# mfinzi/depth-estimation

Hardware: AMD Instinct MI355X
Metric: Mpixel-labels/s per CRF mean-field iter (splat+blur+slice) (higher is better)
Workload: dtype f32; 1 GPU; c3: synthetic 2048x1536x256 cost volume, d=5 bilateral features (BASELINE configs[2]); H=1536, W=2048, L=256, d=5, features=synthetic smooth colours sigma_xy=8.0 sigma_c=0.1, n=3145728, M=296893, parallelism=single GPU, launch=eager, arithmetic=default (fp32-rounding-equivalent, ~1e-7 rel), table=reference

## Files before the change

### depth-estimation_amd/csrc/phl_api.hip

```cpp
#include <math.h>
#include <stdarg.h>
#include <stdio.h>
#include <string.h>

#include <map>
#include <chrono>
#include <mutex>
#include <utility>
#include <vector>

#include "phl_internal.h"

namespace {
thread_local char g_err[512] = "";

struct device_guard {
    int prev = -1;
    bool ok = false;
    explicit device_guard(int dev)
    {
        if (hipGetDevice(&prev) != hipSuccess) prev = -1;
        ok = (prev == dev) || (hipSetDevice(dev) == hipSuccess);
    }
    ~device_guard()
// ... 757 lines not shown
int phl_splat_part_pack(phl_lattice *lat, const float *src, int vd, int64_t src_rs, float *vert, float *partial_dev,
                        const int32_t *chunks_dev, int64_t nchunks_sel, const int32_t *rows_dev, int64_t nrows,
                        const int32_t *pack_pos_dev, float *pack_dev, int64_t pack_rs, phl_stream st)
{
    if (!lat || vd < 0 || nchunks_sel < 0 || nrows < 0 || !vert || (nchunks_sel > 0 && (!chunks_dev || !src)) || (nrows > 0 && !rows_dev) ||
        (lat->S_multi > 0 && !partial_dev) || (pack_pos_dev && (!pack_dev || pack_rs < vd || pack_rs % 4 || !phl_al16(pack_dev)))) {
        phl_set_error("phl_splat_part_pack: bad arguments");
        return PHL_ERR_INVALID;
    }
    return splat_subset("phl_splat_part_pack", lat, src, vd, src_rs, vert, partial_dev, chunks_dev, nchunks_sel, rows_dev, nrows,
                        pack_pos_dev, pack_dev, pack_rs, st);
}

int phl_blur_axis(phl_lattice *lat, int axis, const float *vin, float *vout, int vd, phl_stream st)
{
    if (!lat || axis < 0 || axis > lat->d || vd < 0 || vin == vout) { phl_set_error("phl_blur_axis: bad arguments"); return PHL_ERR_INVALID; }
    device_guard g(lat->device);
    return phl_launch_blur(lat, axis, vin, vout, vd, (hipStream_t)st);
}

static int blur_all(const phl_lattice *lat, float *const buf[2], int vd, hipStream_t st, int *cur_out)
{
    static const bool pairs = !(getenv("PHL_BLUR_PAIRS") && atoi(getenv("PHL_BLUR_PAIRS")) == 0);
    int cur = 0;
    for (int axis = 0; axis <= lat->d;) {
        int rc;
        if (pairs && axis + 1 <= lat->d && lat->nbr2) {
            rc = phl_launch_blur2(lat, axis / 2, buf[cur], buf[cur ^ 1], vd, st, true);
            axis += 2;
        } else {
            rc = phl_launch_blur(lat, axis, buf[cur], buf[cur ^ 1], vd, st, true);
            axis += 1;
        }
        if (rc) return rc;
        cur ^= 1;
    }
    *cur_out = cur;
    return PHL_OK;
}

int phl_blur(phl_lattice *lat, float *vert_a, float *vert_b, int vd, int *result_in_b, phl_stream st)
{
    if (!lat || vd < 0 || !result_in_b || vert_a == vert_b || (lat->M > 0 && vd > 0 && (!vert_a || !vert_b))) {
        phl_set_error("phl_blur: bad arguments");
        return PHL_ERR_INVALID;
    }
    device_guard g(lat->device);
// ... 229 lines not shown
    if (lat->M == 0) return PHL_OK;
    device_guard g(lat->device);
    PHL_HIP(hipDeviceSynchronize());
    std::vector<int32_t> f, r;
    int rc = fetch_maps(lat, f, r);
    if (rc) return rc;
    const size_t M = (size_t)lat->M;
    const int axes = lat->d + 1;
    if (r.empty()) {
        PHL_HIP(hipMemcpy(nbr, lat->nbr, sizeof(int32_t) * M * axes * 2, hipMemcpyDeviceToHost));
        return PHL_OK;
    }
    std::vector<int32_t> h(M * axes * 2);
    PHL_HIP(hipMemcpy(h.data(), lat->nbr, sizeof(int32_t) * h.size(), hipMemcpyDeviceToHost));
    for (int a = 0; a < axes; a++)
        for (size_t v = 0; v < M; v++)
            for (int s2 = 0; s2 < 2; s2++) {
                const int32_t x = h[((size_t)a * M + r[v]) * 2 + s2];
                nbr[((size_t)a * M + v) * 2 + s2] = x < 0 ? x : f[x];
            }
    return PHL_OK;
}

int phl_get_splat_lists(phl_lattice *lat, int32_t *ptr, int32_t *pixel, float *w)
{
    if (!lat || !ptr || !pixel || !w) { phl_set_error("phl_get_splat_lists: bad arguments"); return PHL_ERR_INVALID; }
    if (lat->N == 0) { ptr[0] = 0; return PHL_OK; }
    device_guard g(lat->device);
    const int rc0 = phl_ensure_csr(lat, nullptr);
    if (rc0) return rc0;
    std::vector<phl_contrib_t> h((size_t)lat->N);
    std::vector<int32_t> p((size_t)lat->M + 1);
    PHL_HIP(hipDeviceSynchronize());
    PHL_HIP(hipMemcpy(p.data(), lat->csr_ptr, sizeof(int32_t) * p.size(), hipMemcpyDeviceToHost));
    PHL_HIP(hipMemcpy(h.data(), lat->csr, sizeof(phl_contrib_t) * h.size(), hipMemcpyDeviceToHost));
    std::vector<int32_t> f, r;
    int rc = fetch_maps(lat, f, r);
    if (rc) return rc;
    int64_t o = 0;
    for (int64_t v = 0; v < lat->M; v++) {
        const int64_t row = r.empty() ? v : r[v];
        ptr[v] = (int32_t)o;
        for (int32_t e = p[row]; e < p[row + 1]; e++, o++) { pixel[o] = h[e].pixel; w[o] = h[e].w; }
    }
    ptr[lat->M] = (int32_t)o;
    return PHL_OK;
// ... 4 lines not shown
```

### depth-estimation_amd/csrc/phl_build.hip

```cpp
#include <cstring>
#include <mutex>

#include "phl_device_utils.h"

namespace {

struct sf_t {
    float v[PHL_MAX_D];
};

template <int D>
struct pix_rec {
    static constexpr int GW = (D + 1) / 2;
    static constexpr int W = GW + (D + 5) / 6;
    static __device__ __forceinline__ void load(const uint32_t *__restrict__ p, uint32_t (&w)[W])
    {
        if constexpr (W == 4) {
            const uint4 v = *reinterpret_cast<const uint4 *>(p);
            w[0] = v.x; w[1] = v.y; w[2] = v.z; w[3] = v.w;
        } else if constexpr (W == 2) {
            const uint2 v = *reinterpret_cast<const uint2 *>(p);
            w[0] = v.x; w[1] = v.y;
        } else {
#pragma unroll
// ... 392 lines not shown
        for (int side = 0; side < 2; side++) t[side] = open[side] ? table[h[side]] : PHL_EMPTY;
        uint32_t other[2][K::KW];
#pragma unroll
        for (int side = 0; side < 2; side++) {
            if (t[side] == PHL_EMPTY) { open[side] = false; continue; }
            K::load(vkp + (int64_t)(-(t[side] + 1)) * K::PW, other[side]);
        }
#pragma unroll
        for (int side = 0; side < 2; side++) {
            if (!open[side]) continue;
            bool same = true;
#pragma unroll
            for (int j = 0; j < K::KW; j++) same &= (other[side][j] == want[side][j]);
            if (same) { res[side] = -(t[side] + 1); open[side] = false; }
            else h[side] = (h[side] + 1) & mask;
        }
    }
    nbr[idx * 2 + 0] = res[0];
    nbr[idx * 2 + 1] = res[1];
}

template <int D>
int launch_neighbors(const int16_t *vkeys, int M, const int *table, uint32_t mask, int *nbr, phl_dev_block<uint32_t> &scratch,
                     hipStream_t st)
{
    using K = packed_key<D>;
    PHL_TRY(scratch.alloc((size_t)M * K::PW + 4));
    uint32_t *const vkp = scratch.get();
    hipLaunchKernelGGL(k_pack_keys<D>, dim3((M + 255) / 256), dim3(256), 0, st, vkeys, M, vkp);
    const int64_t tot = (int64_t)M * (D + 1);
    hipLaunchKernelGGL(k_neighbors<D>, dim3((unsigned)((tot + 255) / 256)), dim3(256), 0, st, vkp, M, table, mask, nbr);
    PHL_HIP(hipGetLastError());
    return PHL_OK;
}

__global__ __launch_bounds__(256) void k_compose_pairs(const int2 *__restrict__ nbr, int M, int npairs, int4 *__restrict__ nbr2)
{
    const int64_t idx = (int64_t)blockIdx.x * blockDim.x + threadIdx.x;
    if (idx >= (int64_t)M * npairs) return;
    const int p = (int)(idx / M);
    const int v = (int)(idx - (int64_t)p * M);
    const int2 *na = nbr + (int64_t)(2 * p) * M;
    const int2 nb = nbr[(int64_t)(2 * p + 1) * M + v];
    const int2 none = make_int2(-1, -1);
    const int2 am = nb.x >= 0 ? na[nb.x] : none;
    const int2 a0 = na[v];
    const int2 ap = nb.y >= 0 ? na[nb.y] : none;
    nbr2[idx * 2 + 0] = make_int4(am.x, nb.x, am.y, a0.x);
    nbr2[idx * 2 + 1] = make_int4(a0.y, ap.x, nb.y, ap.y);
}

struct hidden_t {
    int n;
    int32_t id[PHL_MAX_HIDDEN];
};

__global__ __launch_bounds__(256) void k_table_insert(const int16_t *__restrict__ vkeys, int d, int M, int *table,
                                                      uint32_t mask, hidden_t hidden, const int *__restrict__ int_of_ft)
{
    const int v = blockIdx.x * blockDim.x + threadIdx.x;
    if (v >= M) return;
    for (int i = 0; i < hidden.n; i++)
        if ((int_of_ft ? int_of_ft[hidden.id[i]] : hidden.id[i]) == v) return;
    const int16_t *key = vkeys + (int64_t)v * d;
    uint32_t h = mix_begin();
    for (int i = 0; i < d; i++) h = mix_step(h, key[i]);
    h = mix_end(h) & mask;
    while (atomicCAS(&table[h], PHL_EMPTY, -(v + 1)) != PHL_EMPTY) h = (h + 1) & mask;
}

__global__ __launch_bounds__(256) void k_table_lookup(const int16_t *__restrict__ qkeys, int d, int K,
                                                      const int16_t *__restrict__ vkeys, const int *__restrict__ table,
// ... 115 lines not shown

#define PHL_FOR_D(X)                                                                                                     \
    X(1) X(2) X(3) X(4) X(5) X(6) X(7) X(8) X(9) X(10) X(11) X(12) X(13) X(14) X(15) X(16)

__global__ __launch_bounds__(256) void k_iota_from(int *p, int n, int first)
{
    const int i = blockIdx.x * blockDim.x + threadIdx.x;
    if (i < n) p[i] = first + i;
}

__global__ void k_override_nbr00(int *nbr, const int *__restrict__ int_of_ft, int value)
{
    const int row = int_of_ft ? int_of_ft[0] : 0;
    nbr[(int64_t)row * 2] = (value >= 0 && int_of_ft) ? int_of_ft[value] : value;
}

}

int phl_rebuild_table_and_neighbors(phl_lattice *lat, hipStream_t st, phl_dev_block<uint32_t> &scratch)
{
    const int d = lat->d;
    const int M = (int)lat->M;
    PHL_HIP(phl_lat_free(lat->nbr2));
    uint64_t cap = 1024;
    while (cap < (uint64_t)M * 2) cap <<= 1;
    lat->table_mask = (uint32_t)(cap - 1);
    PHL_HIP(phl_lat_alloc(lat->table, cap));
    PHL_HIP(phl_lat_alloc(lat->nbr, (size_t)M * (d + 1) * 2));
    hipLaunchKernelGGL(k_fill_i32, dim3(1024), dim3(256), 0, st, lat->table, (int64_t)cap, PHL_EMPTY);
    if (M > 0) {
        hidden_t hidden;
        hidden.n = lat->n_hidden;
        for (int i = 0; i < lat->n_hidden; i++) hidden.id[i] = lat->hidden[i];
        hipLaunchKernelGGL(k_table_insert, dim3((M + 255) / 256), dim3(256), 0, st, lat->vkeys, d, M, lat->table,
                           lat->table_mask, hidden, lat->int_of_ft);
        int rcn = PHL_OK;
        switch (d) {
#define PHL_CASE(D) case D: rcn = launch_neighbors<D>(lat->vkeys, M, lat->table, lat->table_mask, lat->nbr, scratch, st); break;
            PHL_FOR_D(PHL_CASE)
#undef PHL_CASE
        }
        if (rcn) return rcn;
        if (lat->nbr00_override != -2)
            hipLaunchKernelGGL(k_override_nbr00, dim3(1), dim3(1), 0, st, lat->nbr, lat->int_of_ft, lat->nbr00_override);
        const int npairs = (d + 1) / 2;
        PHL_HIP(phl_lat_alloc(lat->nbr2, (size_t)M * npairs * 8));
        const int64_t totp = (int64_t)M * npairs;
        hipLaunchKernelGGL(k_compose_pairs, dim3((unsigned)((totp + 255) / 256)), dim3(256), 0, st,
                           reinterpret_cast<const int2 *>(lat->nbr), M, npairs, reinterpret_cast<int4 *>(lat->nbr2));
    }
    PHL_HIP(hipGetLastError());
    return PHL_OK;
}

int phl_write_final_vids(phl_lattice *lat, hipStream_t st)
{
    if (!lat->bt_slot_of || !lat->bt_table) { phl_set_error("phl_write_final_vids: no build tables"); return PHL_ERR_INVALID; }
    const int N = (int)lat->N;
    if (N > 0) {
        hipLaunchKernelGGL(k_final_vid, dim3((unsigned)(((int64_t)N + 256 * FV_PER - 1) / (256 * FV_PER))), dim3(256), 0, st, lat->bt_table, lat->bt_slot_of, N,
                           lat->bt_remap, lat->bt_dup_ptr, lat->bt_seg_e, lat->bt_seg_id, lat->int_of_ft, lat->replay);
        PHL_HIP(hipGetLastError());
    }
    return PHL_OK;
}

namespace {
struct side_t {
    int dev = -1;
    hipStream_t s = nullptr;
    hipEvent_t fork = nullptr, join = nullptr;
};
// ... 306 lines not shown
```

### depth-estimation_amd/csrc/phl_filter.hip

```cpp
#include <stdlib.h>

#include <type_traits>

#include "phl_internal.h"

namespace {

template <int VEC> struct vec_of;
template <> struct vec_of<1> { using type = float; };
template <> struct vec_of<4> { using type = float4; };

template <int VEC> __device__ __forceinline__ typename vec_of<VEC>::type vzero();
template <> __device__ __forceinline__ float vzero<1>() { return 0.f; }
template <> __device__ __forceinline__ float4 vzero<4>() { return make_float4(0.f, 0.f, 0.f, 0.f); }

__device__ __forceinline__ float vload(const float *p, float) { return *p; }
__device__ __forceinline__ float4 vload(const float *p, float4) { return *reinterpret_cast<const float4 *>(p); }
__device__ __forceinline__ void vstore(float *p, float v) { *p = v; }
__device__ __forceinline__ void vstore(float *p, float4 v) { *reinterpret_cast<float4 *>(p) = v; }

__device__ __forceinline__ float mac(float acc, float w, float q) { return acc + w * q; }
__device__ __forceinline__ float4 mac(float4 acc, float w, float4 q)
{
    return make_float4(acc.x + w * q.x, acc.y + w * q.y, acc.z + w * q.z, acc.w + w * q.w);
// ... 171 lines not shown
            s[u] = vload(vin + vc * vd + c, V());
#pragma unroll
            for (int k = 0; k < 8; k++) {
                if constexpr (LPR == 64) {
                    const int idk = __builtin_amdgcn_readfirstlane(id[u][k]);
                    x[u][k] = vzero<VEC>();
                    if (idk >= 0) x[u][k] = vload(vin + (int64_t)idk * vd + c, V());
                } else {
                    x[u][k] = vzero<VEC>();
                    if (__ballot(id[u][k] >= 0) != 0ull)
                        x[u][k] = vload(vin + (id[u][k] >= 0 ? (int64_t)id[u][k] : vc) * vd + c, V());
                }
            }
        }
#pragma unroll
        for (int u = 0; u < U; u++) {
#pragma unroll
            for (int k = 0; k < 8; k++)
                if (id[u][k] < 0) x[u][k] = vzero<VEC>();
            const V tm = id[u][1] >= 0 ? blur3(x[u][0], x[u][1], x[u][2]) : vzero<VEC>();
            const V t0 = blur3(x[u][3], s[u], x[u][4]);
            const V tp = id[u][6] >= 0 ? blur3(x[u][5], x[u][6], x[u][7]) : vzero<VEC>();
            if (v[u] < M) vstore(vout + v[u] * vd + c, blur3(tm, t0, tp));
        }
    }
}

template <int VEC, int LPR, bool EXACT>
__global__ __launch_bounds__(256) void k_slice(const float *__restrict__ vert, int vd,
                                               const phl_replay_t *__restrict__ replay, int dp1, int64_t n,
                                               float *__restrict__ out, int64_t out_rs,
                                               const float *__restrict__ sub_src, int64_t sub_rs, float cdiv,
                                               float rcdiv)
{
    using V = typename vec_of<VEC>::type;
    constexpr int G = 64 / LPR;
    const int lane = threadIdx.x & 63;
    const int sub = lane / LPR;
    const int l = lane % LPR;
    const int64_t stride = (int64_t)waves_in_grid() * G;
    for (int64_t p0 = (int64_t)wave_in_grid() * G; p0 < n; p0 += stride) {
        const int64_t p = p0 + sub;
        if (p >= n) continue;
        const phl_replay_t *rp = replay + p * dp1;
        for (int c = l * VEC; c < vd; c += LPR * VEC) {
            V acc = vzero<VEC>();
// ... 185 lines not shown
    });
    PHL_HIP(hipGetLastError());
    return PHL_OK;
}

int phl_launch_rows(bool scatter, float *vert, int vd, const int64_t *idx, int64_t k, float *buf, int64_t buf_rs, hipStream_t st)
{
    if (k == 0 || vd == 0) return PHL_OK;
    if (vd % 4 || buf_rs % 4 || !phl_al16(vert) || !phl_al16(buf)) {
        phl_set_error("row gather/scatter: needs vd %% 4 == 0 and 16-byte aligned rows");
        return PHL_ERR_UNSUPPORTED;
    }
    const int lpr = pick_lpr(vd, 4);
    const unsigned grid = (unsigned)((k + (64 / lpr) * 4 - 1) / ((64 / lpr) * 4));
    dispatch_int<PHL_LPRS>(lpr, [&](auto L) {
        constexpr int LPR = decltype(L)::value;
        if (scatter) k_scatter_add_rows<LPR><<<dim3(grid), dim3(256), 0, st>>>(vert, vd, idx, k, buf, buf_rs);
        else k_gather_rows<LPR><<<dim3(grid), dim3(256), 0, st>>>(vert, vd, idx, k, buf, buf_rs);
    });
    PHL_HIP(hipGetLastError());
    return PHL_OK;
}

int phl_launch_blur2(const phl_lattice *lat, int pair, const float *vin, float *vout, int vd, hipStream_t st, bool restricted)
{
    const int M = (int)lat->M;
    if (M == 0 || vd == 0) return PHL_OK;
    const blur_rows_t rr = rows_of(lat, 2 * pair + 1, restricted);
    if (rr.total == 0) return PHL_OK;
    const int4 *nb2 = reinterpret_cast<const int4 *>(lat->nbr2) + (int64_t)pair * M * 2;
    const bool v4 = (vd % 4 == 0) && phl_al16(vin) && phl_al16(vout);
    constexpr int U2 = 1;
    const row_launch rl = launch_rows(rr.total, vd, v4, U2);
    dispatch_int<PHL_LPRS>(rl.lpr, [&](auto L) {
        constexpr int LPR = decltype(L)::value;
        if (v4) k_blur2<4, LPR, U2><<<dim3(rl.grid), dim3(256), 0, st>>>(vin, vout, nb2, M, vd, rl.xcd_chunk, rr);
        else k_blur2<1, LPR, U2><<<dim3(rl.grid), dim3(256), 0, st>>>(vin, vout, nb2, M, vd, rl.xcd_chunk, rr);
    });
    PHL_HIP(hipGetLastError());
    return PHL_OK;
}

int phl_launch_slice(const phl_lattice *lat, const float *vert, int vd, float *out, int64_t out_rs, const float *sub,
                     int64_t sub_rs, unsigned flags, hipStream_t st)
{
    const int64_t n = lat->n;
    if (n == 0 || vd == 0) return PHL_OK;
    const int dp1 = lat->d + 1;
    const float cdiv = 1 + powf(2, -lat->d);
    const float rcdiv = 1.0f / cdiv;
    const bool v4 = (vd % 4 == 0) && (out_rs % 4 == 0) && phl_al16(vert) && phl_al16(out) &&
                    (!sub || ((sub_rs % 4 == 0) && phl_al16(sub)));
    const int lpr = pick_lpr(vd, v4 ? 4 : 1);
// ... 48 lines not shown
```

### depth-estimation_amd/csrc/phl_internal.h

```cpp
#pragma once
#include <hip/hip_runtime.h>
#include <stdint.h>
#include <stdlib.h>

#include "phl.h"

#include <type_traits>
#include <utility>
#include <vector>

#define PHL_WAVE 64
#define PHL_MAX_HIDDEN 64
#define PHL_EMPTY 0x7FFFFFFF

void phl_set_error(const char *fmt, ...);
int phl_hip_fail(hipError_t e, const char *what, const char *file, int line);
#define PHL_HIP(call)                                                              \
    do {                                                                           \
        hipError_t e__ = (call);                                                   \
        if (e__ != hipSuccess) return phl_hip_fail(e__, #call, __FILE__, __LINE__); \
    } while (0)
#define PHL_TRY(call) \
    do { const int rc__ = (call); if (rc__ != PHL_OK) return rc__; } while (0)

struct phl_replay_t {
    int32_t vid;
    float w;
};
struct phl_contrib_t {
    int32_t pixel;
    float w;
};

struct phl_lattice {
    int device;
    int d;
    int64_t n;
    int64_t M;
    int64_t N;

    int16_t *vkeys;
    phl_replay_t *replay;
    int32_t *csr_ptr;
    phl_contrib_t *csr;
    int32_t *nbr;
    int32_t *nbr2;
    int *table;
    uint32_t table_mask;
    int64_t M_local;
    int32_t *vfirst;
    int64_t vfirst_valid_for_M;
    int32_t *bt_slot_of, *bt_table;
    int32_t *bt_remap, *bt_dup_ptr, *bt_seg_e, *bt_seg_id;
    int32_t *bt_cell;
    int grid_nca, grid_ncb;
    int32_t *ft_of_int;
    int32_t *int_of_ft;

    int P;
    int nchunks;
    int nv_max;
    int64_t S;
    int64_t S_multi;
    int32_t *pix_order;
    int32_t *chunk_vptr;
    int32_t *slot_vert;
    int32_t *slot_pidx;
    int2 *seg_rng;
    phl_contrib_t *seg;
// ... 21 lines not shown
    int32_t nbr00_override;
};

hipError_t phl_dev_malloc(void **p, size_t bytes);
hipError_t phl_dev_free(void *p);

template <typename T>
inline hipError_t phl_lat_free(T *&member) { return phl_dev_free(std::exchange(member, nullptr)); }
template <typename T>
inline hipError_t phl_lat_alloc(T *&member, size_t count)
{
    hipError_t e = phl_lat_free(member);
    void *p = nullptr;
    if (e == hipSuccess) e = phl_dev_malloc(&p, sizeof(T) * (count ? count : (size_t)1));
    if (e == hipSuccess) member = (T *)p;
    return e;
}

template <typename... T>
inline void phl_lat_free_all(T *&...member) { ((void)phl_lat_free(member), ...); }
inline void phl_lat_free_persistent(phl_lattice *lat)
{
    phl_lat_free_all(lat->vkeys, lat->replay, lat->csr_ptr, lat->csr, lat->nbr, lat->nbr2, lat->table, lat->ft_of_int, lat->int_of_ft,
                     lat->vfirst);
}
inline void phl_tiles_free(phl_lattice *lat)
{
    phl_lat_free_all(lat->pix_order, lat->chunk_vptr, lat->slot_vert, lat->slot_pidx, lat->seg_rng, lat->seg, lat->lidx, lat->vs_ptr,
                     lat->vs, lat->vorder, lat->chunk_by_nv, lat->vlong);
    free(lat->nv_cum);
    lat->nv_cum = nullptr;
    lat->n_long = lat->S = lat->S_multi = 0;
    lat->nchunks = lat->nv_max = 0;
}
inline void phl_release_build_tables(phl_lattice *lat)
{
    phl_lat_free_all(lat->bt_slot_of, lat->bt_table, lat->bt_remap, lat->bt_dup_ptr, lat->bt_cell);
    lat->bt_seg_e = lat->bt_seg_id = nullptr;
}

struct phl_reftable_query {
    virtual int vid_at(int64_t candidate) = 0;
    virtual int64_t next_occurrence(int clean_vid, int64_t after) = 0;
    virtual void probe_paths_submit(int64_t n_clean, const std::vector<int32_t> &extra_clean,
                                    const std::vector<int32_t> &stale_clean, uint64_t cap,
                                    const std::vector<int32_t> &check) = 0;
    virtual int probe_paths_all_ok() = 0;
// ... 192 lines not shown
struct phl_splat_opts {
    bool subset = false;
    const int *chunk_list = nullptr;
    int nlist = 0;
    const int *vlist = nullptr;
    int64_t nvl = 0;
    const phl_splat_wide *wide = nullptr;
    const int *pack_pos = nullptr;
    float *pack = nullptr;
    int64_t pack_rs = 0;
};
int phl_launch_splat_tiled(phl_lattice *lat, const float *src, int64_t src_rs, int vd, float *vert, float *partial,
                           hipStream_t st, const phl_splat_opts &o = {});
int phl_launch_slice_grad(const phl_lattice *lat, const float *vertw, int L, const float *y, int64_t y_rs, const float *ref,
                          int64_t ref_rs, int64_t ref_cs, float *grad_ref, int k0, int ncols, int accumulate, float *wx_out,
                          int64_t wx_rs, hipStream_t st);
int phl_tiles_chunks_touching(phl_lattice *lat, const int64_t *rows_dev, int64_t k, int32_t *mask_host, hipStream_t st);
int phl_launch_slice_tiled(const phl_lattice *lat, const float *vert, int vd, float *out, int64_t out_rs, const float *sub,
                           int64_t sub_rs, unsigned flags, hipStream_t st);

int phl_launch_splat(phl_lattice *lat, const float *src, int64_t src_rs, int vd, float *vert, hipStream_t st);
int phl_launch_blur(const phl_lattice *lat, int axis, const float *vin, float *vout, int vd, hipStream_t st, bool restricted = false);
int phl_launch_blur2(const phl_lattice *lat, int pair, const float *vin, float *vout, int vd, hipStream_t st, bool restricted = false);
int phl_launch_rows(bool scatter, float *vert, int vd, const int64_t *idx, int64_t k, float *buf, int64_t buf_rs, hipStream_t st);
int phl_launch_slice(const phl_lattice *lat, const float *vert, int vd, float *out, int64_t out_rs,
                     const float *sub, int64_t sub_rs, unsigned flags, hipStream_t st);
int phl_launch_copy2d(const float *src, int64_t srs, int64_t scs, float *dst, int64_t drs, int64_t dcs,
                      int64_t rows, int cols, hipStream_t st);

size_t phl_compat_wide_planes_bytes(int L);
int phl_compat_wide_prepare(const float *mu_t, int L, void *planes, hipStream_t st);
int phl_compat_wide_softmax(const float *E0, int64_t e_rs, const float *X, int64_t x_rs, const float *mu_t, const void *planes,
                            float *out, int64_t o_rs, int64_t n, int L, bool logits, hipStream_t st);
```

### depth-estimation_amd/csrc/phl_tiles_build.hip

```cpp
#include <math.h>
#include <stdio.h>
#include <stdlib.h>

#include <vector>

#include "phl_device_utils.h"

namespace {

__global__ __launch_bounds__(256) void k_minmax(const float *__restrict__ ref, int64_t rs, int64_t cs, int64_t n, int d,
                                                float *__restrict__ out )
{
    __shared__ float smin[4][PHL_MAX_D], smax[4][PHL_MAX_D];
    const int lane = threadIdx.x & 63, w = threadIdx.x >> 6;
    float lo[PHL_MAX_D], hi[PHL_MAX_D];
#pragma unroll
    for (int i = 0; i < PHL_MAX_D; i++) { lo[i] = INFINITY; hi[i] = -INFINITY; }
    for (int64_t p = (int64_t)blockIdx.x * blockDim.x + threadIdx.x; p < n; p += (int64_t)gridDim.x * blockDim.x) {
#pragma unroll
        for (int i = 0; i < PHL_MAX_D; i++)
            if (i < d) {
                const float v = ref[p * rs + i * cs];
                lo[i] = fminf(lo[i], v);
                hi[i] = fmaxf(hi[i], v);
// ... 887 lines not shown
            if (nv_max > NVC) {
                PHL_CHUNK_SORT(true, lat->pix_order, n, P, dp1, lat->replay, (int *)nullptr, lat->chunk_vptr, 0, lat->slot_vert,
                               lat->seg_rng, lat->seg, lat->lidx, (const int *)nv, NVC)
            }
        } else {
            PHL_CHUNK_SORT(true, lat->pix_order, n, P, dp1, lat->replay, (int *)nullptr, lat->chunk_vptr, 0, lat->slot_vert,
                           lat->seg_rng, lat->seg, lat->lidx, (const int *)nullptr, 0)
        }
    }
#undef PHL_CHUNK_SORT
#undef PHL_CHUNK_MASKS
#undef PHL_CHUNK_MASKS_X
    PHL_HIP(hipGetLastError());
    PHL_HIP(nbr_chain.join(st));
    PHL_HIP(hipStreamSynchronize(st));
    }
    phl_release_build_tables(lat);
    PHL_TRY(phl_tiles_link_vertices(lat, st));
    PHL_TRY(vkeys_old.drop());
    PHL_TRY(vfirst_old.drop());
    PHL_TRY(nbr_scratch.drop());
    lat->table_bytes = (int64_t)(sizeof(int16_t) * (size_t)lat->M * d + sizeof(phl_replay_t) * (size_t)N +
                                 sizeof(int32_t) * (size_t)lat->M * (d + 1) * 2 + sizeof(int32_t) * (size_t)lat->M * ((d + 1) / 2) * 8 +
                                 sizeof(int) * ((size_t)lat->table_mask + 1) + (lat->int_of_ft ? 2 * sizeof(int) * (size_t)lat->M : 0));
    lat->tile_bytes = (int64_t)(sizeof(int) * ((size_t)n + nchunks + 1 + 3 * ((size_t)S + 1) + (size_t)lat->M + 1) +
                                sizeof(phl_contrib_t) * ((size_t)N + S + 1) + sizeof(unsigned short) * (size_t)N);
    return PHL_OK;
}

__global__ __launch_bounds__(256) void k_mark_chunks(const int64_t *__restrict__ rows, int64_t k, const int *__restrict__ vs_ptr,
                                                     const phl_contrib_t *__restrict__ vs, const int *__restrict__ chunk_vptr,
                                                     int nchunks, int *__restrict__ mask)
{
    const int64_t i = (int64_t)blockIdx.x * blockDim.x + threadIdx.x;
    if (i >= k) return;
    const int64_t v = rows[i];
    for (int e = vs_ptr[v]; e < vs_ptr[v + 1]; e++) {
        const int slot = vs[e].pixel;
        int lo = 0, hi = nchunks - 1;
        while (lo < hi) {
            const int mid = (lo + hi + 1) >> 1;
            if (chunk_vptr[mid] <= slot) lo = mid;
            else hi = mid - 1;
        }
        mask[lo] = 1;
    }
}
// ... 19 lines not shown
```

### depth-estimation_amd/phl/__init__.py

```python
import ctypes as C
import os
import threading
from collections import OrderedDict

import numpy as np
import torch

_HERE = os.path.dirname(os.path.abspath(__file__))
LIB_PATH = os.environ.get("PHL_LIB") or os.path.join(os.path.dirname(_HERE), "lib", "libphl.so")

SUBTRACT_INPUT = 1
EXACT = 4
NO_TILES = 8
ERR_UNSUPPORTED = 7
FILTER_GRAD_MAX_D = 16
GUIDED_FULL_MAX_CX = 4
GUIDED_BILINEAR_FULL_COV = 1
BUILD_REFERENCE_TABLE = 1

_lib = None
_lib_lock = threading.Lock()


class PhlError(RuntimeError):
# ... 64 lines not shown
    ("phl_cost_volume_nchw", "i", "PPiiiiqqqqiiiIPqqqS"),
    ("phl_disparity_wta", "i", "PPiiiiqqqqiiiPPqqS"),
    ("phl_box_blur", "i", "PPqqqiiS"),
    ("phl_box_blur_grad", "i", "PPqqqidPPS"),
    ("phl_box_blur_fused_max_r", "i", "iii"),
    ("phl_guided_filter", "i", "PPPPiiiiiiiiPPPPPfS"),
    ("phl_guided_filter_full", "i", "PPPPiiiiiiiiPPPPPfS"),
    ("phl_guided_filter_max_r", "i", ""),
    ("phl_guided_filter_labels_per_chunk", "i", "iiiiiii"),
    ("phl_guided_filter_grad", "i", "PPPPPPiiiiiiiiPPPPPfiS"),
    ("phl_guided_filter_grad_max_r", "i", ""),
    ("phl_guided_filter_full_grad", "i", "PPPPPPiiiiiiiiPPPPPfiS"),
    ("phl_guided_filter_full_grad_labels_per_chunk", "i", "iiiiiii"),
    ("phl_guided_filter_bilinear", "i", "PPPPiiiiiiiiPfIS"),
    ("phl_guided_filter_bilinear_labels_per_chunk", "i", "iiiii"),
    ("phl_stream_copy", "i", "PPqS"),
    ("phl_copy2d", "i", "PqqPqqqiS"),
    ("phl_tile_stats", "i", "PiP"),
    ("phl_get_vertex_order", "i", "PP"),
    ("phl_get_pixel_order", "i", "PP"),
    ("phl_get_keys", "i", "PP"),
    ("phl_get_replay", "i", "PPP"),
    ("phl_get_neighbors", "i", "PP"),
    ("phl_get_splat_lists", "i", "PPPP"),
    ("phl_debug_reference_table", "i", "PPqiqPqPPPiPP"),
    ("phl_debug_probe_paths", "i", "PqiPiPiQPiiP"),
    ("phl_debug_slow_copy", "i", "PPqiiS"),
    ("phl_debug_side_streams", "i", ""),
    ("phl_debug_live_blocks", "q", ""),
)


def load_library():
    global _lib
    with _lib_lock:
        if _lib is not None:
            return _lib
        if not os.path.exists(LIB_PATH):
            raise RuntimeError(
                f"{LIB_PATH} not found: the HIP extension is not built (run `python __graft_entry__.py`). "
                "There is no CPU fallback for the lattice filter.")
        lib = C.CDLL(LIB_PATH)
        for name, ret, args in _ABI:
            fn = getattr(lib, name, None)
            if fn is not None:
                fn.restype, fn.argtypes = _KINDS[ret], [_KINDS[k] for k in args]
# ... 272 lines not shown
        out.index_copy_(0, self.vertex_rows(), vert_ft)
        return out

    def pixel_order(self):
        out = np.empty(self.n, np.int32)
        _call("phl_get_pixel_order", self._h, _host(out))
        return out

    def keys(self):
        out = np.empty((self.M, self.d), np.int16)
        _call("phl_get_keys", self._h, _host(out))
        return out

    def replay(self):
        vid = np.empty((self.n, self.d + 1), np.int32)
        w = np.empty((self.n, self.d + 1), np.float32)
        _call("phl_get_replay", self._h, _host(vid), _host(w))
        return vid, w

    def neighbors(self):
        out = np.empty((self.d + 1, self.M, 2), np.int32)
        _call("phl_get_neighbors", self._h, _host(out))
        return out

    def splat_lists(self):
        ptr = np.empty(self.M + 1, np.int32)
        pix = np.empty(self.n * (self.d + 1), np.int32)
        w = np.empty(self.n * (self.d + 1), np.float32)
        _call("phl_get_splat_lists", self._h, _host(ptr), _host(pix), _host(w))
        return ptr, pix, w


def _rowmajor(t):
    return t.is_cuda and t.dtype == torch.float32 and t.dim() == 2 and t.stride(1) == 1


def _aligned(t):
    return _rowmajor(t) and t.stride(0) % 4 == 0 and t.data_ptr() % 16 == 0


def softmax_neg_add(E0, G=None, out=None):
    if not _rowmajor(E0) or (G is not None and (not _rowmajor(G) or G.shape != E0.shape)):
        raise TypeError("softmax_neg_add: expects fp32 CUDA [n, L] tensors with unit channel stride")
    n, L = E0.shape
    if out is None:
        out = torch.empty((n, L), dtype=torch.float32, device=E0.device)
# ... 963 lines not shown
```

### include/phl.h

```cpp
#ifndef PHL_H
#define PHL_H

#include <stdint.h>

#ifdef __cplusplus
extern "C" {
#endif

#define PHL_VERSION 100

typedef struct phl_lattice phl_lattice;
typedef void *phl_stream;

enum phl_status {
    PHL_OK = 0,
    PHL_ERR_INVALID = 1,
    PHL_ERR_SHAPE = 2,
    PHL_ERR_HIP = 3,
    PHL_ERR_NO_DEVICE = 4,
    PHL_ERR_KEY_RANGE = 5,
    PHL_ERR_TOO_LARGE = 6,
    PHL_ERR_UNSUPPORTED = 7
};

// ... 172 lines not shown
int phl_guided_filter_full_grad(const float *y_dev, const float *x_dev, const float *g_dev, float *grad_y_dev, float *grad_x_dev,
                                float *grad_eps_dev, int B, int cy, int cx, int H, int W, int h, int w, int r,
                                const int *row_of_low_dev, const int *col_of_low_dev, const int *low_of_row_dev,
                                const int *low_of_col_dev, const float *eps_dev, float scale, int subtract_is_y, phl_stream stream);
int phl_guided_filter_full_grad_labels_per_chunk(int B, int cy, int cx, int h, int w, int full, int needs);

#define PHL_GUIDED_BILINEAR_FULL_COV 1u
int phl_guided_filter_bilinear(const float *y_dev, const float *x_dev, const float *src_dev, float *out_dev, int B, int cy, int cx,
                               int H, int W, int h, int w, int r, const float *eps_dev, float scale, unsigned flags,
                               phl_stream stream);
int phl_guided_filter_bilinear_labels_per_chunk(int B, int cy, int cx, int h, int w);

int phl_stream_copy(const float *src_dev, float *dst_dev, int64_t n_floats, phl_stream stream);
int phl_copy2d(const float *src_dev, int64_t src_row_stride, int64_t src_col_stride, float *dst_dev, int64_t dst_row_stride,
               int64_t dst_col_stride, int64_t rows, int cols, phl_stream stream);

int phl_tile_stats(const phl_lattice *lat, int vd, int64_t out[7]);

int phl_get_vertex_order(phl_lattice *lat, int32_t *row_of_vertex_host );
int phl_get_pixel_order(phl_lattice *lat, int32_t *pix_order_host );
int phl_get_keys(phl_lattice *lat, int16_t *keys_host );
int phl_get_replay(phl_lattice *lat, int32_t *vid_host , float *w_host );
int phl_get_neighbors(phl_lattice *lat, int32_t *nbr_host );
int phl_get_splat_lists(phl_lattice *lat, int32_t *ptr_host , int32_t *pixel_host ,
                        float *w_host );

int phl_debug_reference_table(const int16_t *keys_clean, const int32_t *cand_vid, int64_t M, int d, int64_t N,
                              int16_t *keys_ref_out, int64_t keys_ref_cap, int64_t *M_ref_out,
                              int32_t *cand_ref_vid_out, int32_t *hidden_out, int hidden_cap, int *n_hidden_out,
                              int *blur_first_nbr_out);

int phl_debug_probe_paths(const int16_t *keys_clean, int64_t n_clean, int d, const int32_t *extra_clean, int n_extra,
                          const int32_t *stale_clean, int n_stale, uint64_t cap, const int32_t *check, int n_check,
                          int on_device, int *result_out);

int phl_debug_slow_copy(const float *src_dev, float *dst_dev, int64_t n_floats, int workgroups, int repeat, phl_stream stream);
int phl_debug_side_streams(void);
int64_t phl_debug_live_blocks(void);

#ifdef __cplusplus
}
#endif
#endif
```

Before: 384,500 Mpixel-labels/s.

## Fuse three blur axes per pass using precomputed line lists with sliding reuse

Adds a triple-axis blur kernel. It walks precomputed lines along the third axis of each group and reuses the pair-blurred values of the previous and next vertices as a sliding window. With d=5 this covers the six axes as two triple passes instead of three pair passes. The intent is fewer full passes over the vertex buffer and less global memory traffic. In exchange, lattice build gets extra line-construction kernels and tables, a single wave handles each short line serially, and neighbours at item cuts need redundant evaluation.

```diff
diff --git a/depth-estimation_amd/csrc/phl_api.hip b/depth-estimation_amd/csrc/phl_api.hip
--- a/depth-estimation_amd/csrc/phl_api.hip
+++ b/depth-estimation_amd/csrc/phl_api.hip
@@ -803,7 +803,18 @@
 static int blur_all(const phl_lattice *lat, float *const buf[2], int vd, hipStream_t st, int *cur_out)
 {
     static const bool pairs = !(getenv("PHL_BLUR_PAIRS") && atoi(getenv("PHL_BLUR_PAIRS")) == 0);
+    static const bool triples = !(getenv("PHL_BLUR_TRIPLES") && atoi(getenv("PHL_BLUR_TRIPLES")) == 0);
     int cur = 0;
+    if (pairs && triples && phl_blur3_takes(lat, buf[0], buf[1], vd)) {
+        for (int slot = 0; slot < lat->np3; slot++) {
+            const int rc = slot < lat->n3 ? phl_launch_blur3(lat, slot, buf[cur], buf[cur ^ 1], vd, st)
+                                          : phl_launch_blur2_slot(lat, slot, buf[cur], buf[cur ^ 1], vd, st);
+            if (rc) return rc;
+            cur ^= 1;
+        }
+        *cur_out = cur;
+        return PHL_OK;
+    }
     for (int axis = 0; axis <= lat->d;) {
         int rc;
         if (pairs && axis + 1 <= lat->d && lat->nbr2) {
@@ -1079,6 +1090,36 @@
     return PHL_OK;
 }
 
+int phl_get_blur_lines(phl_lattice *lat, int group, int32_t *vertex, int32_t *flags, int32_t *item_start, int64_t info[3])
+{
+    if (!lat || !info) { phl_set_error("phl_get_blur_lines: bad arguments"); return PHL_ERR_INVALID; }
+    const bool have = lat->lines && lat->line_items && lat->n3 > 0;
+    info[0] = have ? lat->n3 : 0;
+    info[1] = have ? lat->nitems3 : 0;
+    info[2] = have ? lat->line_item_size : 0;
+    if (!vertex && !flags && !item_start) return PHL_OK;
+    if (!have || group < 0 || group >= lat->n3 || !vertex || !flags || !item_start) {
+        phl_set_error("phl_get_blur_lines: no line list for group %d", group);
+        return PHL_ERR_INVALID;
+    }
+    device_guard g(lat->device);
+    PHL_HIP(hipDeviceSynchronize());
+    std::vector<int32_t> f, r;
+    int rc = fetch_maps(lat, f, r);
+    if (rc) return rc;
+    const size_t M = (size_t)lat->M;
+    std::vector<uint32_t> h(M);
+    PHL_HIP(hipMemcpy(h.data(), lat->lines + (size_t)group * M, sizeof(uint32_t) * M, hipMemcpyDeviceToHost));
+    PHL_HIP(hipMemcpy(item_start, lat->line_items + (size_t)group * (lat->nitems3 + 1), sizeof(int32_t) * (size_t)(lat->nitems3 + 1),
+                      hipMemcpyDeviceToHost));
+    for (size_t i = 0; i < M; i++) {
+        const uint32_t row = h[i] & PHL_LINE_VERTEX;
+        vertex[i] = (f.empty() || row >= M) ? (int32_t)row : f[row];
+        flags[i] = (int32_t)(h[i] >> 28);
+    }
+    return PHL_OK;
+}
+
 int phl_get_splat_lists(phl_lattice *lat, int32_t *ptr, int32_t *pixel, float *w)
 {
     if (!lat || !ptr || !pixel || !w) { phl_set_error("phl_get_splat_lists: bad arguments"); return PHL_ERR_INVALID; }
diff --git a/depth-estimation_amd/csrc/phl_build.hip b/depth-estimation_amd/csrc/phl_build.hip
--- a/depth-estimation_amd/csrc/phl_build.hip
+++ b/depth-estimation_amd/csrc/phl_build.hip
@@ -438,11 +438,13 @@
 
 template <int D>
 int launch_neighbors(const int16_t *vkeys, int M, const int *table, uint32_t mask, int *nbr, phl_dev_block<uint32_t> &scratch,
-                     hipStream_t st)
+                     size_t extra_words, uint32_t **extra, hipStream_t st)
 {
     using K = packed_key<D>;
-    PHL_TRY(scratch.alloc((size_t)M * K::PW + 4));
+    const size_t own = ((size_t)M * K::PW + 4 + 3) / 4 * 4;
+    PHL_TRY(scratch.alloc(own + extra_words));
     uint32_t *const vkp = scratch.get();
+    *extra = vkp + own;
     hipLaunchKernelGGL(k_pack_keys<D>, dim3((M + 255) / 256), dim3(256), 0, st, vkeys, M, vkp);
     const int64_t tot = (int64_t)M * (D + 1);
     hipLaunchKernelGGL(k_neighbors<D>, dim3((unsigned)((tot + 255) / 256)), dim3(256), 0, st, vkp, M, table, mask, nbr);
@@ -464,6 +466,82 @@
     const int2 ap = nb.y >= 0 ? na[nb.y] : none;
     nbr2[idx * 2 + 0] = make_int4(am.x, nb.x, am.y, a0.x);
     nbr2[idx * 2 + 1] = make_int4(a0.y, ap.x, nb.y, ap.y);
+}
+
+struct pair_axes_t {
+    int a[PHL_MAX_D + 1];
+};
+__global__ __launch_bounds__(256) void k_compose_pairs_at(const int2 *__restrict__ nbr, int M, int nslots, pair_axes_t ax,
+                                                          int4 *__restrict__ out)
+{
+    const int64_t idx = (int64_t)blockIdx.x * blockDim.x + threadIdx.x;
+    if (idx >= (int64_t)M * nslots) return;
+    const int j = (int)(idx / M);
+    const int v = (int)(idx - (int64_t)j * M);
+    const int2 *na = nbr + (int64_t)ax.a[j] * M;
+    const int2 nb = nbr[(int64_t)(ax.a[j] + 1) * M + v];
+    const int2 none = make_int2(-1, -1);
+    const int2 am = nb.x >= 0 ? na[nb.x] : none;
+    const int2 a0 = na[v];
+    const int2 ap = nb.y >= 0 ? na[nb.y] : none;
+    out[idx * 2 + 0] = make_int4(am.x, nb.x, am.y, a0.x);
+    out[idx * 2 + 1] = make_int4(a0.y, ap.x, nb.y, ap.y);
+}
+
+__global__ __launch_bounds__(256) void k_line_len(const int2 *__restrict__ nbr, int M, int n3, int *__restrict__ len)
+{
+    const int64_t idx = (int64_t)blockIdx.x * blockDim.x + threadIdx.x;
+    if (idx >= (int64_t)M * n3) return;
+    const int g = (int)(idx / M);
+    const int v = (int)(idx - (int64_t)g * M);
+    const int2 *nc = nbr + (int64_t)(3 * g + 2) * M;
+    const int p = nc[v].x;
+    int l = 0;
+    if (!(p >= 0 && nc[p].y == v)) {
+        int u = v;
+        for (l = 1; l < M; l++) {
+            const int w = nc[u].y;
+            if (w < 0 || nc[w].x != u) break;
+            u = w;
+        }
+    }
+    len[idx] = l;
+}
+
+__device__ __forceinline__ bool line_cut_at(int p, int s, int l, int K, int M)
+{
+    return p > s && p % K == 0 && s + l >= (p + K < M ? p + K : M);
+}
+__global__ __launch_bounds__(256) void k_line_fill(const int2 *__restrict__ nbr, int M, int n3, int K, int nitems,
+                                                   const int *__restrict__ len, const int *__restrict__ pos,
+                                                   uint32_t *__restrict__ lines, int *__restrict__ items)
+{
+    const int64_t idx = (int64_t)blockIdx.x * blockDim.x + threadIdx.x;
+    if (idx >= (int64_t)M * n3) return;
+    const int l = len[idx];
+    if (l == 0) return;
+    const int g = (int)(idx / M);
+    const int2 *nc = nbr + (int64_t)(3 * g + 2) * M;
+    const int s = pos[idx] - g * M;
+    if (s < 0 || s + l > M) return;
+    atomicMin(&items[(int64_t)g * (nitems + 1) + s / K], s);
+    int u = (int)(idx - (int64_t)g * M);
+    for (int o = 0; o < l; o++) {
+        const int p = s + o;
+        const int2 nb = nc[u];
+        const uint32_t fm = nb.x < 0 ? PHL_LINE_ABSENT : ((o > 0 && !line_cut_at(p, s, l, K, M)) ? PHL_LINE_SLIDE : PHL_LINE_EVAL);
+        const uint32_t fp = nb.y < 0 ? PHL_LINE_ABSENT : ((o + 1 < l && !line_cut_at(p + 1, s, l, K, M)) ? PHL_LINE_SLIDE : PHL_LINE_EVAL);
+        lines[(int64_t)g * M + p] = (uint32_t)u | (fm << 28) | (fp << 30);
+        u = nb.y;
+    }
+}
+__global__ __launch_bounds__(256) void k_line_items_finish(int M, int n3, int K, int nitems, int *__restrict__ items)
+{
+    const int64_t idx = (int64_t)blockIdx.x * blockDim.x + threadIdx.x;
+    if (idx >= (int64_t)(nitems + 1) * n3) return;
+    const int b = (int)(idx % (nitems + 1));
+    if (b == nitems) items[idx] = M;
+    else if (items[idx] == 0x7FFFFFFF) items[idx] = b * K;
 }
 
 struct hidden_t {
@@ -625,6 +703,19 @@
     const int d = lat->d;
     const int M = (int)lat->M;
     PHL_HIP(phl_lat_free(lat->nbr2));
+    PHL_HIP(phl_lat_free(lat->nbr3));
+    PHL_HIP(phl_lat_free(lat->lines));
+    PHL_HIP(phl_lat_free(lat->line_items));
+    lat->n3 = lat->np3 = 0;
+    lat->nitems3 = 0;
+    static const int line_item = getenv("PHL_BLUR3_ITEM") ? atoi(getenv("PHL_BLUR3_ITEM")) : 4;
+    const int naxes = d + 1;
+    const int n3 = naxes % 3 == 1 ? naxes / 3 - 1 : naxes / 3;
+    const bool ghosts = lat->M_local > 0 && lat->M_local < lat->M;
+    const bool triples = n3 > 0 && !ghosts && M > 0 && (int64_t)M <= (int64_t)PHL_LINE_VERTEX && (int64_t)M * n3 < ((int64_t)1 << 30) &&
+                         line_item >= 1 && line_item <= 32;
+    const size_t line_words = triples ? 2 * (size_t)M * n3 + (size_t)M * n3 / SCAN_TILE + 16 : 0;
+    uint32_t *line_tmp = nullptr;
     uint64_t cap = 1024;
     while (cap < (uint64_t)M * 2) cap <<= 1;
     lat->table_mask = (uint32_t)(cap - 1);
@@ -639,7 +730,7 @@
                            lat->table_mask, hidden, lat->int_of_ft);
         int rcn = PHL_OK;
         switch (d) {
-#define PHL_CASE(D) case D: rcn = launch_neighbors<D>(lat->vkeys, M, lat->table, lat->table_mask, lat->nbr, scratch, st); break;
+#define PHL_CASE(D) case D: rcn = launch_neighbors<D>(lat->vkeys, M, lat->table, lat->table_mask, lat->nbr, scratch, line_words, &line_tmp, st); break;
             PHL_FOR_D(PHL_CASE)
 #undef PHL_CASE
         }
@@ -651,6 +742,33 @@
         const int64_t totp = (int64_t)M * npairs;
         hipLaunchKernelGGL(k_compose_pairs, dim3((unsigned)((totp + 255) / 256)), dim3(256), 0, st,
                            reinterpret_cast<const int2 *>(lat->nbr), M, npairs, reinterpret_cast<int4 *>(lat->nbr2));
+        if (triples) {
+            pair_axes_t ax = {};
+            int np3 = 0;
+            for (int g = 0; g < n3; g++) ax.a[np3++] = 3 * g;
+            for (int a = 3 * n3; a + 1 < naxes; a += 2) ax.a[np3++] = a;
+            const int K = line_item;
+            const int nitems = (M + K - 1) / K;
+            PHL_HIP(phl_lat_alloc(lat->nbr3, (size_t)M * np3 * 8));
+            PHL_HIP(phl_lat_alloc(lat->lines, (size_t)M * n3));
+            PHL_HIP(phl_lat_alloc(lat->line_items, (size_t)(nitems + 1) * n3));
+            const int2 *nbr = reinterpret_cast<const int2 *>(lat->nbr);
+            int *const len = reinterpret_cast<int *>(line_tmp), *const pos = len + (size_t)M * n3, *const tile_sums = pos + (size_t)M * n3 + 1;
+            const int64_t tot3 = (int64_t)M * n3;
+            const unsigned g3 = (unsigned)((tot3 + 255) / 256);
+            hipLaunchKernelGGL(k_compose_pairs_at, dim3((unsigned)(((int64_t)M * np3 + 255) / 256)), dim3(256), 0, st, nbr, M, np3, ax,
+                               reinterpret_cast<int4 *>(lat->nbr3));
+            hipLaunchKernelGGL(k_line_len, dim3(g3), dim3(256), 0, st, nbr, M, n3, len);
+            hipLaunchKernelGGL(k_fill_i32, dim3(256), dim3(256), 0, st, lat->line_items, (int64_t)(nitems + 1) * n3, 0x7FFFFFFF);
+            PHL_TRY(exclusive_scan(len, pos, (int)tot3, tile_sums, st));
+            hipLaunchKernelGGL(k_line_fill, dim3(g3), dim3(256), 0, st, nbr, M, n3, K, nitems, len, pos, lat->lines, lat->line_items);
+            hipLaunchKernelGGL(k_line_items_finish, dim3((unsigned)(((int64_t)(nitems + 1) * n3 + 255) / 256)), dim3(256), 0, st, M, n3, K,
+                               nitems, lat->line_items);
+            lat->n3 = n3;
+            lat->np3 = np3;
+            lat->nitems3 = nitems;
+            lat->line_item_size = K;
+        }
     }
     PHL_HIP(hipGetLastError());
     return PHL_OK;
diff --git a/depth-estimation_amd/csrc/phl_filter.hip b/depth-estimation_amd/csrc/phl_filter.hip
--- a/depth-estimation_amd/csrc/phl_filter.hip
+++ b/depth-estimation_amd/csrc/phl_filter.hip
@@ -217,6 +217,83 @@
             const V t0 = blur3(x[u][3], s[u], x[u][4]);
             const V tp = id[u][6] >= 0 ? blur3(x[u][5], x[u][6], x[u][7]) : vzero<VEC>();
             if (v[u] < M) vstore(vout + v[u] * vd + c, blur3(tm, t0, tp));
+        }
+    }
+}
+
+struct pair_ids_t {
+    int id[8];
+};
+__device__ __forceinline__ pair_ids_t load_pair_ids(const int4 *__restrict__ nb2, int u)
+{
+    const int4 i0 = nb2[(int64_t)u * 2], i1 = nb2[(int64_t)u * 2 + 1];
+    const int raw[8] = {i0.x, i0.y, i0.z, i0.w, i1.x, i1.y, i1.z, i1.w};
+    pair_ids_t r;
+#pragma unroll
+    for (int k = 0; k < 8; k++) r.id[k] = __builtin_amdgcn_readfirstlane(raw[k]);
+    return r;
+}
+template <int VEC>
+__device__ __forceinline__ typename vec_of<VEC>::type blur2_value(const float *__restrict__ vin, const pair_ids_t &I, int u, int vd, int c)
+{
+    using V = typename vec_of<VEC>::type;
+    V x[8];
+    const V s = vload(vin + (int64_t)u * vd + c, V());
+#pragma unroll
+    for (int k = 0; k < 8; k++) {
+        x[k] = vzero<VEC>();
+        if (I.id[k] >= 0) x[k] = vload(vin + (int64_t)I.id[k] * vd + c, V());
+    }
+    const V tm = I.id[1] >= 0 ? blur3(x[0], x[1], x[2]) : vzero<VEC>();
+    const V t0 = blur3(x[3], s, x[4]);
+    const V tp = I.id[6] >= 0 ? blur3(x[5], x[6], x[7]) : vzero<VEC>();
+    return blur3(tm, t0, tp);
+}
+
+template <int VEC>
+__global__ __launch_bounds__(256) void k_blur3(const float *__restrict__ vin, float *__restrict__ vout,
+                                               const int4 *__restrict__ nb2, const int2 *__restrict__ nbc,
+                                               const uint32_t *__restrict__ lines, const int *__restrict__ items, int nitems,
+                                               int M, int vd, int xcd_chunk)
+{
+    using V = typename vec_of<VEC>::type;
+    const int lane = threadIdx.x & 63;
+    const int lb = xcd_chunk > 0 ? (int)(blockIdx.x & 7) * xcd_chunk + (int)(blockIdx.x >> 3) : (int)blockIdx.x;
+    const int wv = lb * 4 + __builtin_amdgcn_readfirstlane((int)(threadIdx.x >> 6));
+    if (wv >= nitems) return;
+    const int e0 = __builtin_amdgcn_readfirstlane(items[wv]);
+    const int cnt = __builtin_amdgcn_readfirstlane(items[wv + 1]) - e0;
+    if (e0 < 0 || cnt <= 0 || cnt > 64 || e0 + cnt > M) return;
+    uint32_t my_ent = lines[e0 + (lane < cnt ? lane : cnt - 1)];
+    if ((int)(my_ent & PHL_LINE_VERTEX) >= M) my_ent = (my_ent & ~PHL_LINE_VERTEX) | (uint32_t)(M - 1);
+    for (int c = lane * VEC; c < vd; c += 64 * VEC) {
+        uint32_t ent = __builtin_amdgcn_readlane(my_ent, 0);
+        int u = (int)(ent & PHL_LINE_VERTEX);
+        int u1 = (int)(__builtin_amdgcn_readlane(my_ent, cnt > 1 ? 1 : 0) & PHL_LINE_VERTEX);
+        pair_ids_t I1 = load_pair_ids(nb2, u);
+        V t_prev = vzero<VEC>(), t_cur = blur2_value<VEC>(vin, I1, u, vd, c), t_next = vzero<VEC>();
+        I1 = load_pair_ids(nb2, u1);
+        for (int i = 0; i < cnt; i++) {
+            const uint32_t ent1 = __builtin_amdgcn_readlane(my_ent, i + 1 < cnt ? i + 1 : i);
+            if (i + 1 < cnt) t_next = blur2_value<VEC>(vin, I1, u1, vd, c);
+            const int u2 = (int)(__builtin_amdgcn_readlane(my_ent, i + 2 < cnt ? i + 2 : i) & PHL_LINE_VERTEX);
+            if (i + 2 < cnt) I1 = load_pair_ids(nb2, u2);
+            const uint32_t fm = (ent >> 28) & 3u, fp = ent >> 30;
+            V tm = vzero<VEC>(), tp = vzero<VEC>();
+            if (fm == PHL_LINE_SLIDE) tm = t_prev;
+            if (fp == PHL_LINE_SLIDE) tp = t_next;
+            if (fm == PHL_LINE_EVAL || fp == PHL_LINE_EVAL) {
+                const int2 nc = nbc[u];
+                const int um = __builtin_amdgcn_readfirstlane(nc.x), up = __builtin_amdgcn_readfirstlane(nc.y);
+                if (fm == PHL_LINE_EVAL && um >= 0) tm = blur2_value<VEC>(vin, load_pair_ids(nb2, um), um, vd, c);
+                if (fp == PHL_LINE_EVAL && up >= 0) tp = blur2_value<VEC>(vin, load_pair_ids(nb2, up), up, vd, c);
+            }
+            vstore(vout + (int64_t)u * vd + c, blur3(tm, t_cur, tp));
+            t_prev = t_cur;
+            t_cur = t_next;
+            ent = ent1;
+            u = u1;
+            u1 = u2;
         }
     }
 }
@@ -448,13 +525,60 @@
     return PHL_OK;
 }
 
+static int launch_blur2_table(const phl_lattice *lat, const int4 *nb2, const blur_rows_t &rr, const float *vin, float *vout, int vd,
+                              hipStream_t st);
+
 int phl_launch_blur2(const phl_lattice *lat, int pair, const float *vin, float *vout, int vd, hipStream_t st, bool restricted)
 {
     const int M = (int)lat->M;
     if (M == 0 || vd == 0) return PHL_OK;
     const blur_rows_t rr = rows_of(lat, 2 * pair + 1, restricted);
     if (rr.total == 0) return PHL_OK;
-    const int4 *nb2 = reinterpret_cast<const int4 *>(lat->nbr2) + (int64_t)pair * M * 2;
+    return launch_blur2_table(lat, reinterpret_cast<const int4 *>(lat->nbr2) + (int64_t)pair * M * 2, rr, vin, vout, vd, st);
+}
+
+int phl_launch_blur2_slot(const phl_lattice *lat, int slot, const float *vin, float *vout, int vd, hipStream_t st)
+{
+    const int M = (int)lat->M;
+    if (M == 0 || vd == 0) return PHL_OK;
+    if (!lat->nbr3 || slot < 0 || slot >= lat->np3) { phl_set_error("phl_launch_blur2_slot: no pair table %d", slot); return PHL_ERR_INVALID; }
+    const blur_rows_t rr = rows_of(lat, 0, false);
+    return launch_blur2_table(lat, reinterpret_cast<const int4 *>(lat->nbr3) + (int64_t)slot * M * 2, rr, vin, vout, vd, st);
+}
+
+bool phl_blur3_takes(const phl_lattice *lat, const float *vin, const float *vout, int vd)
+{
+    if (!lat->lines || !lat->nbr3 || !lat->line_items || lat->n3 <= 0 || lat->blur_rows_set) return false;
+    const bool v4 = (vd % 4 == 0) && phl_al16(vin) && phl_al16(vout);
+    return pick_lpr(vd, v4 ? 4 : 1) == 64;
+}
+
+int phl_launch_blur3(const phl_lattice *lat, int group, const float *vin, float *vout, int vd, hipStream_t st)
+{
+    const int M = (int)lat->M;
+    if (M == 0 || vd == 0) return PHL_OK;
+    if (!phl_blur3_takes(lat, vin, vout, vd) || group < 0 || group >= lat->n3) {
+        phl_set_error("phl_launch_blur3: no line lists for group %d at vd = %d", group, vd);
+        return PHL_ERR_INVALID;
+    }
+    const int nitems = (int)lat->nitems3;
+    const int4 *nb2 = reinterpret_cast<const int4 *>(lat->nbr3) + (int64_t)group * M * 2;
+    const int2 *nbc = reinterpret_cast<const int2 *>(lat->nbr) + (int64_t)(3 * group + 2) * M;
+    const uint32_t *lines = lat->lines + (int64_t)group * M;
+    const int *items = lat->line_items + (int64_t)group * (nitems + 1);
+    const bool v4 = (vd % 4 == 0) && phl_al16(vin) && phl_al16(vout);
+    int xcd_chunk;
+    const unsigned grid = phl_xcd_grid(((int64_t)nitems + 3) / 4, &xcd_chunk);
+    if (v4) k_blur3<4><<<dim3(grid), dim3(256), 0, st>>>(vin, vout, nb2, nbc, lines, items, nitems, M, vd, xcd_chunk);
+    else k_blur3<1><<<dim3(grid), dim3(256), 0, st>>>(vin, vout, nb2, nbc, lines, items, nitems, M, vd, xcd_chunk);
+    PHL_HIP(hipGetLastError());
+    return PHL_OK;
+}
+
+static int launch_blur2_table(const phl_lattice *lat, const int4 *nb2, const blur_rows_t &rr, const float *vin, float *vout, int vd,
+                              hipStream_t st)
+{
+    const int M = (int)lat->M;
     const bool v4 = (vd % 4 == 0) && phl_al16(vin) && phl_al16(vout);
     constexpr int U2 = 1;
     const row_launch rl = launch_rows(rr.total, vd, v4, U2);
diff --git a/depth-estimation_amd/csrc/phl_internal.h b/depth-estimation_amd/csrc/phl_internal.h
--- a/depth-estimation_amd/csrc/phl_internal.h
+++ b/depth-estimation_amd/csrc/phl_internal.h
@@ -12,6 +12,10 @@
 #define PHL_WAVE 64
 #define PHL_MAX_HIDDEN 64
 #define PHL_EMPTY 0x7FFFFFFF
+#define PHL_LINE_ABSENT 0u
+#define PHL_LINE_SLIDE 1u
+#define PHL_LINE_EVAL 2u
+#define PHL_LINE_VERTEX 0x0FFFFFFFu
 
 void phl_set_error(const char *fmt, ...);
 int phl_hip_fail(hipError_t e, const char *what, const char *file, int line);
@@ -45,6 +49,11 @@
     phl_contrib_t *csr;
     int32_t *nbr;
     int32_t *nbr2;
+    int32_t *nbr3;
+    uint32_t *lines;
+    int32_t *line_items;
+    int n3, np3, line_item_size;
+    int64_t nitems3;
     int *table;
     uint32_t table_mask;
     int64_t M_local;
@@ -112,7 +121,7 @@
 inline void phl_lat_free_persistent(phl_lattice *lat)
 {
     phl_lat_free_all(lat->vkeys, lat->replay, lat->csr_ptr, lat->csr, lat->nbr, lat->nbr2, lat->table, lat->ft_of_int, lat->int_of_ft,
-                     lat->vfirst);
+                     lat->vfirst, lat->nbr3, lat->lines, lat->line_items);
 }
 inline void phl_tiles_free(phl_lattice *lat)
 {
@@ -351,6 +360,9 @@
 int phl_launch_splat(phl_lattice *lat, const float *src, int64_t src_rs, int vd, float *vert, hipStream_t st);
 int phl_launch_blur(const phl_lattice *lat, int axis, const float *vin, float *vout, int vd, hipStream_t st, bool restricted = false);
 int phl_launch_blur2(const phl_lattice *lat, int pair, const float *vin, float *vout, int vd, hipStream_t st, bool restricted = false);
+bool phl_blur3_takes(const phl_lattice *lat, const float *vin, const float *vout, int vd);
+int phl_launch_blur3(const phl_lattice *lat, int group, const float *vin, float *vout, int vd, hipStream_t st);
+int phl_launch_blur2_slot(const phl_lattice *lat, int slot, const float *vin, float *vout, int vd, hipStream_t st);
 int phl_launch_rows(bool scatter, float *vert, int vd, const int64_t *idx, int64_t k, float *buf, int64_t buf_rs, hipStream_t st);
 int phl_launch_slice(const phl_lattice *lat, const float *vert, int vd, float *out, int64_t out_rs,
                      const float *sub, int64_t sub_rs, unsigned flags, hipStream_t st);
diff --git a/depth-estimation_amd/csrc/phl_tiles_build.hip b/depth-estimation_amd/csrc/phl_tiles_build.hip
--- a/depth-estimation_amd/csrc/phl_tiles_build.hip
+++ b/depth-estimation_amd/csrc/phl_tiles_build.hip
@@ -933,7 +933,8 @@
     PHL_TRY(nbr_scratch.drop());
     lat->table_bytes = (int64_t)(sizeof(int16_t) * (size_t)lat->M * d + sizeof(phl_replay_t) * (size_t)N +
                                  sizeof(int32_t) * (size_t)lat->M * (d + 1) * 2 + sizeof(int32_t) * (size_t)lat->M * ((d + 1) / 2) * 8 +
-                                 sizeof(int) * ((size_t)lat->table_mask + 1) + (lat->int_of_ft ? 2 * sizeof(int) * (size_t)lat->M : 0));
+                                 sizeof(int) * ((size_t)lat->table_mask + 1) + (lat->int_of_ft ? 2 * sizeof(int) * (size_t)lat->M : 0) +
+                                 sizeof(int32_t) * ((size_t)lat->M * (8 * lat->np3 + lat->n3) + (size_t)(lat->nitems3 + 1) * lat->n3));
     lat->tile_bytes = (int64_t)(sizeof(int) * ((size_t)n + nchunks + 1 + 3 * ((size_t)S + 1) + (size_t)lat->M + 1) +
                                 sizeof(phl_contrib_t) * ((size_t)N + S + 1) + sizeof(unsigned short) * (size_t)N);
     return PHL_OK;
diff --git a/depth-estimation_amd/phl/__init__.py b/depth-estimation_amd/phl/__init__.py
--- a/depth-estimation_amd/phl/__init__.py
+++ b/depth-estimation_amd/phl/__init__.py
@@ -110,6 +110,7 @@
     ("phl_get_keys", "i", "PP"),
     ("phl_get_replay", "i", "PPP"),
     ("phl_get_neighbors", "i", "PP"),
+    ("phl_get_blur_lines", "i", "PiPPPP"),
     ("phl_get_splat_lists", "i", "PPPP"),
     ("phl_debug_reference_table", "i", "PPqiqPqPPPiPP"),
     ("phl_debug_probe_paths", "i", "PqiPiPiQPiiP"),
@@ -428,6 +429,18 @@
         out = np.empty((self.d + 1, self.M, 2), np.int32)
         _call("phl_get_neighbors", self._h, _host(out))
         return out
+
+    def blur_lines(self, group=None):
+        info = np.zeros(3, np.int64)
+        if group is None:
+            _call("phl_get_blur_lines", self._h, 0, None, None, None, _host(info))
+            return dict(zip(("groups", "items", "item_size"), (int(x) for x in info)))
+        items = self.blur_lines()["items"]
+        vertex = np.empty(self.M, np.int32)
+        flags = np.empty(self.M, np.int32)
+        start = np.empty(items + 1, np.int32)
+        _call("phl_get_blur_lines", self._h, int(group), _host(vertex), _host(flags), _host(start), _host(info))
+        return vertex, flags & 3, (flags >> 2) & 3, start
 
     def splat_lists(self):
         ptr = np.empty(self.M + 1, np.int32)
diff --git a/include/phl.h b/include/phl.h
--- a/include/phl.h
+++ b/include/phl.h
@@ -218,6 +218,8 @@
 int phl_get_keys(phl_lattice *lat, int16_t *keys_host );
 int phl_get_replay(phl_lattice *lat, int32_t *vid_host , float *w_host );
 int phl_get_neighbors(phl_lattice *lat, int32_t *nbr_host );
+int phl_get_blur_lines(phl_lattice *lat, int group, int32_t *vertex_host , int32_t *flags_host ,
+                       int32_t *item_start_host , int64_t info[3]);
 int phl_get_splat_lists(phl_lattice *lat, int32_t *ptr_host , int32_t *pixel_host ,
                         float *w_host );
 
```

Measured after the change: 403,000 Mpixel-labels/s (median of 6 runs). 4.8% higher.
